# tpfeifle/pointcloud-segmentation-attention

Hardware: AMD Instinct MI355X
Metric: 8192-pt clouds/sec through SA+FP layers, 1/2/4/8 MI355X; HBM GB/s vs peak (higher is better)
Workload: dtype f32

## Files before the change

pointcloud-segmentation-attention_amd/csrc/interp.hip:

```cpp
#include <algorithm>
#include <type_traits>

#include "grid.h"

namespace pn2 {
namespace {

constexpr int kNNBlock = 256;
constexpr int kNNGroup = 4;
constexpr int kNNRows = kNNBlock / kNNGroup;
constexpr int kNNTile = 2048;

struct Best3 {
  float d1, d2, d3;
  int i1, i2, i3;
};

PN2_DEV void best3_init(Best3& b) {
  b.d1 = b.d2 = b.d3 = __builtin_inff();
  b.i1 = b.i2 = b.i3 = 0;
}

PN2_DEV void best3_insert(Best3& b, float d, int k) {
  const bool c1 = d < b.d1, c2 = d < b.d2, c3 = d < b.d3;
  b.d3 = c2 ? b.d2 : (c3 ? d : b.d3);
  b.i3 = c2 ? b.i2 : (c3 ? k : b.i3);
  b.d2 = c1 ? b.d1 : (c2 ? d : b.d2);
  b.i2 = c1 ? b.i1 : (c2 ? k : b.i2);
  b.d1 = c1 ? d : b.d1;
  b.i1 = c1 ? k : b.i1;
}

PN2_DEV bool lex_lt(float d, int k, float bd, int bk) { return d < bd || (d == bd && k < bk); }
PN2_DEV void best3_insert_lex(Best3& b, float d, int k) {
  const bool c1 = lex_lt(d, k, b.d1, b.i1), c2 = lex_lt(d, k, b.d2, b.i2),
             c3 = lex_lt(d, k, b.d3, b.i3);
  b.d3 = c2 ? b.d2 : (c3 ? d : b.d3);
  b.i3 = c2 ? b.i2 : (c3 ? k : b.i3);
  b.d2 = c1 ? b.d1 : (c2 ? d : b.d2);
  b.i2 = c1 ? b.i1 : (c2 ? k : b.i2);
  b.d1 = c1 ? d : b.d1;
  b.i1 = c1 ? k : b.i1;
}

PN2_DEV void best3_merge_xor(Best3& b, int mask) {
  const float d1 = __shfl_xor(b.d1, mask, kWave), d2 = __shfl_xor(b.d2, mask, kWave),
              d3 = __shfl_xor(b.d3, mask, kWave);
  const int i1 = __shfl_xor(b.i1, mask, kWave), i2 = __shfl_xor(b.i2, mask, kWave),
            i3 = __shfl_xor(b.i3, mask, kWave);
  best3_insert_lex(b, d1, i1);
  best3_insert_lex(b, d2, i2);
  best3_insert_lex(b, d3, i3);
}

struct Best3K {
  uint64_t k1, k2, k3;
};
PN2_DEV uint64_t nn_key(float d, int k) {
  return ((uint64_t)__float_as_uint(d) << 32) | (uint32_t)k;
}
PN2_DEV void best3k_init(Best3K& b) { b.k1 = b.k2 = b.k3 = nn_key(__builtin_inff(), 0); }
PN2_DEV void best3k_insert(Best3K& b, uint64_t key) {
  const bool c1 = key < b.k1, c2 = key < b.k2, c3 = key < b.k3;
  b.k3 = c2 ? b.k2 : (c3 ? key : b.k3);
  b.k2 = c1 ? b.k1 : (c2 ? key : b.k2);
  b.k1 = c1 ? key : b.k1;
}
template <int CTRL>
PN2_DEV uint64_t quad_xor_u64(uint64_t v) {
  const uint32_t lo = dpp_u32<CTRL>((uint32_t)v);
  const uint32_t hi = dpp_u32<CTRL>((uint32_t)(v >> 32));
  return ((uint64_t)hi << 32) | lo;
}
template <int CTRL>
PN2_DEV void best3k_merge_quad(Best3K& b) {
  const uint64_t o1 = quad_xor_u64<CTRL>(b.k1), o2 = quad_xor_u64<CTRL>(b.k2),
                 o3 = quad_xor_u64<CTRL>(b.k3);
  best3k_insert(b, o1);
  best3k_insert(b, o2);
  best3k_insert(b, o3);
}
PN2_DEV Best3 best3_of(const Best3K& b) {
  Best3 r;
  r.d1 = __uint_as_float((uint32_t)(b.k1 >> 32));
  r.d2 = __uint_as_float((uint32_t)(b.k2 >> 32));
  r.d3 = __uint_as_float((uint32_t)(b.k3 >> 32));
  r.i1 = (int)(uint32_t)b.k1;
  r.i2 = (int)(uint32_t)b.k2;
  r.i3 = (int)(uint32_t)b.k3;
  return r;
}

PN2_DEV void scan_known(const float* __restrict__ K, int m, float x1, float y1, float z1,
                        float4* sk, Best3& best, int tile = kNNTile) {
  const int q = threadIdx.x & (kNNGroup - 1);
  for (int t0 = 0; t0 < m; t0 += tile) {
    const int cnt = min(tile, m - t0);
    __syncthreads();
    for (int e = threadIdx.x; e < cnt; e += kNNBlock) {
      const float* p = K + 3 * (size_t)(t0 + e);
      sk[e] = make_float4(p[0], p[1], p[2], 0.0f);
    }
    __syncthreads();
#pragma unroll 8
    for (int e = q; e < cnt; e += kNNGroup) {
      const float4 p = sk[e];
      best3_insert(best, sqdist(p.x, p.y, p.z, x1, y1, z1), t0 + e);
    }
  }
  best3_merge_xor(best, 1);
  best3_merge_xor(best, 2);
}

__global__ __launch_bounds__(kNNBlock) void three_nn_kernel(const float* __restrict__ xyz1,
                                                            const float* __restrict__ xyz2, int n,
                                                            int m, float* __restrict__ dist,
                                                            int32_t* __restrict__ idx) {
  __shared__ float4 sk[kNNTile];
  const int b = blockIdx.y;
  const int j = blockIdx.x * kNNRows + threadIdx.x / kNNGroup;
  const bool valid = j < n;
  const float* U = xyz1 + ((size_t)b * n + (valid ? j : 0)) * 3;
  Best3 best;
  best3_init(best);
  scan_known(xyz2 + (size_t)b * m * 3, m, U[0], U[1], U[2], sk, best);
  if (valid && (threadIdx.x & (kNNGroup - 1)) == 0) {
    float* D = dist + ((size_t)b * n + j) * 3;
    int32_t* I = idx + ((size_t)b * n + j) * 3;
    D[0] = best.d1; D[1] = best.d2; D[2] = best.d3;
    I[0] = best.i1; I[1] = best.i2; I[2] = best.i3;
  }
}


PN2_DEV bool box_certifies(const GridHdr& h, float px, float py, float pz, int xl, int xh,
                           int yl, int yh, int zl, int zh, float d3) {
  if (!(d3 < __builtin_inff())) return false;
  const float edge = 1.0f / h.inv;
  float gap = __builtin_inff();
  auto face = [&](float d, float pc, float o, int c) {
    const float fc = o + (float)c * edge;
    gap = fminf(gap, d - 1e-5f * (fabsf(pc) + fabsf(o) + fabsf(fc) + (float)c * edge) - 1e-30f);
  };
  if (xl > 0) face(px - (h.ox + (float)xl * edge), px, h.ox, xl);
  if (xh < h.nx - 1) face((h.ox + (float)(xh + 1) * edge) - px, px, h.ox, xh + 1);
  if (yl > 0) face(py - (h.oy + (float)yl * edge), py, h.oy, yl);
  if (yh < h.ny - 1) face((h.oy + (float)(yh + 1) * edge) - py, py, h.oy, yh + 1);
  if (zl > 0) face(pz - (h.oz + (float)zl * edge), pz, h.oz, zl);
  if (zh < h.nz - 1) face((h.oz + (float)(zh + 1) * edge) - pz, pz, h.oz, zh + 1);
  return gap > 0.0f && d3 < gap * gap * 0.9999f;
}

PN2_DEV float axis_gap(float p, float o, float edge, int c, int cp) {
  if (c == cp) return 0.0f;
  const int f = c > cp ? c : c + 1;
  const float fc = o + (float)f * edge;
  const float d = c > cp ? fc - p : p - fc;
  return fmaxf(d - 1e-5f * (fabsf(p) + fabsf(o) + fabsf(fc) + (float)f * edge) - 1e-30f, 0.0f);
}
PN2_DEV bool gap_excludes(float g2, float d3) { return d3 < g2 * 0.9999f; }

constexpr int kNNFirst = 1;

template <int G, typename Off>
PN2_DEV Best3 grid_nn3(const GridHdr& h, const float4* __restrict__ pts,
                       const Off* __restrict__ off, float px, float py, float pz, int q) {
  Best3K best;
  best3k_init(best);
  auto merged = [&]() {
    Best3K mb = best;
    if constexpr (G == 4) {
      best3k_merge_quad<kDppXor1>(mb);
      best3k_merge_quad<kDppXor2>(mb);
    }
    return best3_of(mb);
  };
  const int cx = cell_coord(px, h.ox, h.inv, h.nx);
  const int cy = cell_coord(py, h.oy, h.inv, h.ny);
  const int cz = cell_coord(pz, h.oz, h.inv, h.nz);
  Best3 res;
  for (int s = kNNFirst;; ++s) {
    const int xl = cx - s, xh = cx + s, yl = cy - s, yh = cy + s, zl = cz - s, zh = cz + s;
    const int x0 = max(xl, 0), x1 = min(xh, h.nx - 1);
    const bool block = s == kNNFirst;
    auto visit = [&](int lo, int hi) {
      for (int e = lo + q; e < hi; e += G) {
        const float4 p = pts[e];
        best3k_insert(best, nn_key(sqdist(p.x, p.y, p.z, px, py, pz), __float_as_int(p.w)));
      }
    };
    if (block) {
      for (int z = max(zl, 0); z <= min(zh, h.nz - 1); ++z)
        for (int y = max(yl, 0); y <= min(yh, h.ny - 1); ++y) {
          const int row = (z * h.ny + y) * h.nx;
          visit(off[row + x0], off[row + x1 + 1]);
        }
    } else {
      const float d3 = res.d3, edge = 1.0f / h.inv;
#pragma nounroll
      for (int z = max(zl, 0); z <= min(zh, h.nz - 1); ++z) {
        const float gz = axis_gap(pz, h.oz, edge, z, cz), gz2 = gz * gz;
        if (gap_excludes(gz2, d3)) continue;
#pragma nounroll
        for (int y = max(yl, 0); y <= min(yh, h.ny - 1); ++y) {
          const float gy = axis_gap(py, h.oy, edge, y, cy), gyz = gz2 + gy * gy;
          if (gap_excludes(gyz, d3)) continue;
          const int row = (z * h.ny + y) * h.nx;
          const bool face = z == zl || z == zh || y == yl || y == yh;
          int xa = face ? x0 : xl, xb = face ? x1 : xh;
#pragma nounroll
          while (xa <= xb) {
            const float g = axis_gap(px, h.ox, edge, xa, cx);
            if (xa >= 0 && xa < h.nx && !gap_excludes(gyz + g * g, d3)) break;
            xa = face || xa != xl ? xa + 1 : xh;
          }
#pragma nounroll
          while (xb > xa) {
            const float g = axis_gap(px, h.ox, edge, xb, cx);
            if (xb >= 0 && xb < h.nx && !gap_excludes(gyz + g * g, d3)) break;
            xb = face || xb != xh ? xb - 1 : xl;
          }
          if (xa > xb) continue;
          if (face || xa == xb) {
            visit(off[row + xa], off[row + xb + 1]);
          } else {
            visit(off[row + xa], off[row + xa + 1]);
            visit(off[row + xb], off[row + xb + 1]);
          }
        }
      }
    }
    res = merged();
    if (xl <= 0 && yl <= 0 && zl <= 0 && xh >= h.nx - 1 && yh >= h.ny - 1 && zh >= h.nz - 1)
      break;
    if (box_certifies(h, px, py, pz, xl, xh, yl, yh, zl, zh, res.d3)) break;
  }
  return res;
}

template <int G, typename Off>
PN2_DEV Best3 grid_nn3_wave(const GridHdr& h, const float4* __restrict__ pts,
                            const Off* __restrict__ off, float px, float py, float pz, int q,
                            bool valid) {
  if (valid) return grid_nn3<G, Off>(h, pts, off, px, py, pz, q);
  Best3 none;
  best3_init(none);
  return none;
}


template <int BLOCK, bool LDS, int G, int K>
__global__ __launch_bounds__(BLOCK) void three_nn_grid_kernel(
    const void* __restrict__ kgrid, int m, const void* __restrict__ ugrid,
    const float* __restrict__ xyz1, int n, int B, float* __restrict__ dist,
    int32_t* __restrict__ idx) {
  static_assert(G == 1 || G == 4, "one lane or a quad per unknown");
  constexpr int QPB = BLOCK / G;
  extern __shared__ float4 s_pts[];
  const int R = (n + QPB * K - 1) / (QPB * K);
  const int Lg = xcd_block(blockIdx.x, R * B);
  if (Lg >= R * B) return;
  const int b = Lg / R;
  const int q = (int)threadIdx.x & (G - 1);
  const GridView g = grid_view(kgrid, b, m);
  const GridHdr& h = g.h;
  const float4* __restrict__ pts = g.pts;
  const int* __restrict__ off = g.off;
  if (LDS && h.ncell <= max(m, kAutoMinCells)) {
    int* s_off = (int*)(s_pts + m);
    for (int e = threadIdx.x; e < m; e += BLOCK) s_pts[e] = g.pts[e];
    for (int e = threadIdx.x; e <= h.ncell; e += BLOCK) s_off[e] = g.off[e];
    __syncthreads();
    pts = s_pts;
    off = s_off;
  }
  const float4* __restrict__ upts = ugrid ? grid_view(ugrid, b, n).pts : nullptr;
  for (int kb = 0; kb < K; ++kb) {
    const int i0 = ((Lg - b * R) * K + kb) * QPB;
    if (i0 >= n) break;
    const int i = i0 + (int)threadIdx.x / G;
    const bool valid = i < n;
    const int ic = valid ? i : n - 1;
    float px, py, pz;
    int u;
    if (upts) {
      const float4 U = upts[ic];
      px = U.x; py = U.y; pz = U.z;
      u = __float_as_int(U.w);
    } else {
      const float* U = xyz1 + ((size_t)b * n + ic) * 3;
      px = U[0]; py = U[1]; pz = U[2];
      u = ic;
    }
    const Best3 res = grid_nn3_wave<G, int>(h, pts, off, px, py, pz, q, valid);
    if (valid && q == 0) {
      float* D = dist + ((size_t)b * n + u) * 3;
      int32_t* I = idx + ((size_t)b * n + u) * 3;
      D[0] = res.d1; D[1] = res.d2; D[2] = res.d3;
      I[0] = res.i1; I[1] = res.i2; I[2] = res.i3;
    }
  }
}

__global__ void idw_kernel(const float* __restrict__ dist, int total, float* __restrict__ weight) {
  const int i = blockIdx.x * blockDim.x + threadIdx.x;
  if (i >= total) return;
  const float* d = dist + 3 * (size_t)i;
  float w1, w2, w3;
  idw(d[0], d[1], d[2], w1, w2, w3);
  weight[3 * (size_t)i + 0] = w1;
  weight[3 * (size_t)i + 1] = w2;
  weight[3 * (size_t)i + 2] = w3;
}

constexpr int kBlock = 256;
constexpr int kTileElems = 2048;

__global__ __launch_bounds__(kBlock) void three_interp_kernel(
    const float* __restrict__ points, const int32_t* __restrict__ idx,
    const float* __restrict__ weight, int m, int C, int n, int rows, FastDiv div_c,
    FastDiv div_n, uint32_t total_rows, float* __restrict__ out) {
  const uint32_t r0 = blockIdx.x * (uint32_t)rows;
  const int nrows = (int)min((uint32_t)rows, total_rows - r0);
  const int elems = nrows * C;
  for (int e = threadIdx.x; e < elems; e += kBlock) {
    const uint32_t rl = fdiv((uint32_t)e, div_c);
    const int c = e - (int)rl * C;
    const uint32_t r = r0 + rl;
    const uint32_t b = fdiv(r, div_n);
    const int32_t* I = idx + 3 * (size_t)r;
    const float* W = weight + 3 * (size_t)r;
    const float* P = points + (size_t)b * m * C + c;
    float v = P[(size_t)I[0] * C] * W[0];
    v = v + P[(size_t)I[1] * C] * W[1];
    v = v + P[(size_t)I[2] * C] * W[2];
    out[(size_t)r * C + c] = v;
  }
}

__global__ __launch_bounds__(kBlock) void three_interp_grad_kernel(
    const float* __restrict__ grad_out, const int32_t* __restrict__ idx,
    const float* __restrict__ weight, int m, int C, int rows, FastDiv div_c, FastDiv div_n,
    uint32_t total_rows, float* __restrict__ grad_points) {
  const uint32_t r0 = blockIdx.x * (uint32_t)rows;
  const int nrows = (int)min((uint32_t)rows, total_rows - r0);
  const int elems = nrows * C;
  for (int e = threadIdx.x; e < elems; e += kBlock) {
    const uint32_t rl = fdiv((uint32_t)e, div_c);
    const int c = e - (int)rl * C;
    const uint32_t r = r0 + rl;
    const uint32_t b = fdiv(r, div_n);
    const int32_t* I = idx + 3 * (size_t)r;
    const float* W = weight + 3 * (size_t)r;
    float* G = grad_points + (size_t)b * m * C + c;
    const float g = grad_out[(size_t)r * C + c];
    atomicAdd(G + (size_t)I[0] * C, g * W[0]);
    atomicAdd(G + (size_t)I[1] * C, g * W[1]);
    atomicAdd(G + (size_t)I[2] * C, g * W[2]);
  }
}

struct FpLayer {
  const float* xyz1;
  const float* xyz2;
  const float* pdist;
  const int32_t* pidx;
  const void* ugrid;
  const float* points1;
  const float* points2;
  float* out;
  int C1, C2, n, m, cw, B, Z;
  FastDiv div_cw;
};

struct FpRow {
  int4 I;
  float4 W;
  int r;
};

template <int V2, int V1, int UN, int FB = kNNBlock, typename RowFn>
PN2_DEV void fp_write_rows(const FpLayer& p, int b, int zb, int j0, RowFn row) {
  const float* __restrict__ points1 = p.points1;
  const float* __restrict__ points2 = p.points2;
  float* __restrict__ out = p.out;
  const int C1 = p.C1, C2 = p.C2, n = p.n, m = p.m, cw = p.cw;
  const FastDiv div_cw = p.div_cw;
  const int Cout = C2 + C1;
  const int c2v = C2 / V2, coutv = c2v + C1 / V1;
  const int cb = zb * cw;
  const int ce = min(coutv, cb + cw);
  if (ce <= cb) return;
  const int nrows = min(FB / kNNGroup, n - j0);
  const int elems = nrows * cw;
  using V2T = typename std::conditional<V2 == 4, float4, float>::type;
  using V1T = typename std::conditional<
      V1 == 4, float4, typename std::conditional<V1 == 2, float2, float>::type>::type;
  const V2T* P2 = reinterpret_cast<const V2T*>(points2 + (size_t)b * m * C2);
  const float* P1 = points1 + (size_t)b * n * C1;
  float* O = out + (size_t)b * n * Cout;
  constexpr int U = UN;
  for (int e0 = threadIdx.x; e0 < elems; e0 += FB * U) {
    V2T a[U], bb[U], cc[U];
    V1T q[U];
    float4 W[U];
    bool cat[U], ok[U];
    size_t o[U];
#pragma unroll
    for (int u = 0; u < U; ++u) {
      const int e = e0 + u * FB;
      const int rl = (int)fdiv((uint32_t)(e < elems ? e : e0), div_cw);
      int c = cb + ((e < elems ? e : e0) - rl * cw);
      ok[u] = e < elems && c < ce;
      c = min(c, ce - 1);
      const FpRow rw = row(rl);
      const int r = rw.r;
      cat[u] = c >= c2v;
      W[u] = rw.W;
      if constexpr (V1 == V2) {
        const int4 I = rw.I;
        const V2T* P1v = reinterpret_cast<const V2T*>(P1);
        const V2T* pa = cat[u] ? P1v + (size_t)r * (C1 / V1) + (c - c2v) : P2 + (size_t)I.x * c2v + c;
        const V2T* pb = cat[u] ? pa : P2 + (size_t)I.y * c2v + c;
        const V2T* pc = cat[u] ? pa : P2 + (size_t)I.z * c2v + c;
        a[u] = *pa;
        bb[u] = *pb;
        cc[u] = *pc;
        q[u] = V1T{};
        o[u] = (size_t)r * Cout + (size_t)c * V2;
      } else if (!cat[u]) {
        q[u] = V1T{};
        const int4 I = rw.I;
        a[u] = P2[(size_t)I.x * c2v + c];
        bb[u] = P2[(size_t)I.y * c2v + c];
        cc[u] = P2[(size_t)I.z * c2v + c];
        o[u] = (size_t)r * Cout + (size_t)c * V2;
      } else {
        q[u] = *reinterpret_cast<const V1T*>(P1 + (size_t)r * C1 + (size_t)(c - c2v) * V1);
        a[u] = bb[u] = cc[u] = V2T{};
        o[u] = (size_t)r * Cout + C2 + (size_t)(c - c2v) * V1;
      }
    }
#pragma unroll
    for (int u = 0; u < U; ++u) {
      if (!ok[u]) continue;
      if constexpr (V1 == V2) {
        const bool k = cat[u];
        if constexpr (V2 == 4) {
          float4 v;
          v.x = k ? a[u].x : (a[u].x * W[u].x + bb[u].x * W[u].y) + cc[u].x * W[u].z;
          v.y = k ? a[u].y : (a[u].y * W[u].x + bb[u].y * W[u].y) + cc[u].y * W[u].z;
          v.z = k ? a[u].z : (a[u].z * W[u].x + bb[u].z * W[u].y) + cc[u].z * W[u].z;
          v.w = k ? a[u].w : (a[u].w * W[u].x + bb[u].w * W[u].y) + cc[u].w * W[u].z;
          *reinterpret_cast<float4*>(O + o[u]) = v;
        } else {
          O[o[u]] = k ? a[u] : (a[u] * W[u].x + bb[u] * W[u].y) + cc[u] * W[u].z;
        }
        continue;
      }
      if (cat[u]) {
        *reinterpret_cast<V1T*>(O + o[u]) = q[u];
        continue;
      }
      if constexpr (V2 == 4) {
        float4 v;
        v.x = (a[u].x * W[u].x + bb[u].x * W[u].y) + cc[u].x * W[u].z;
        v.y = (a[u].y * W[u].x + bb[u].y * W[u].y) + cc[u].y * W[u].z;
        v.z = (a[u].z * W[u].x + bb[u].z * W[u].y) + cc[u].z * W[u].z;
        v.w = (a[u].w * W[u].x + bb[u].w * W[u].y) + cc[u].w * W[u].z;
        if (V1 == 4 || (o[u] & 3) == 0) {
          *reinterpret_cast<float4*>(O + o[u]) = v;
        } else if (V1 == 2) {
          *reinterpret_cast<float2*>(O + o[u]) = make_float2(v.x, v.y);
          *reinterpret_cast<float2*>(O + o[u] + 2) = make_float2(v.z, v.w);
        } else {
          O[o[u]] = v.x;
          O[o[u] + 1] = v.y;
          O[o[u] + 2] = v.z;
          O[o[u] + 3] = v.w;
        }
      } else {
        O[o[u]] = (a[u] * W[u].x + bb[u] * W[u].y) + cc[u] * W[u].z;
      }
    }
  }
}

template <int V2, int V1, bool PRE, int UN>
PN2_DEV void fp_fused_body(const FpLayer& p, int Lg, float4* sk, int tile) {
  __shared__ int4 s_idx[kNNRows];
  __shared__ float4 s_w[kNNRows];
  __shared__ int s_row[PRE ? kNNRows : 1];
  const float* __restrict__ xyz1 = p.xyz1;
  const float* __restrict__ xyz2 = p.xyz2;
  const float* __restrict__ pdist = p.pdist;
  const int32_t* __restrict__ pidx = p.pidx;
  const void* __restrict__ ugrid = p.ugrid;
  const int n = p.n, m = p.m, Z = p.Z;
  const int R = (n + kNNRows - 1) / kNNRows;
  const int b = Lg / (R * Z);
  const int zb = (Lg - b * R * Z) / R;
  const int j0 = (Lg - b * R * Z - zb * R) * kNNRows;
  if constexpr (PRE) {
    int jj = j0 + (int)threadIdx.x;
    if (threadIdx.x < kNNRows && jj < n) {
      if (ugrid) jj = __float_as_int(grid_view(ugrid, b, n).pts[jj].w);
      s_row[threadIdx.x] = jj;
      const float* D = pdist + ((size_t)b * n + jj) * 3;
      const int32_t* I = pidx + ((size_t)b * n + jj) * 3;
      float w1, w2, w3;
      idw(D[0], D[1], D[2], w1, w2, w3);
      s_idx[threadIdx.x] = make_int4(I[0], I[1], I[2], 0);
      s_w[threadIdx.x] = make_float4(w1, w2, w3, 0.0f);
    }
  } else {
    const int jl = threadIdx.x / kNNGroup;
    const int j = j0 + jl;
    const bool valid = j < n;
    const float* U = xyz1 + ((size_t)b * n + (valid ? j : 0)) * 3;
    Best3 best;
    best3_init(best);
    scan_known(xyz2 + (size_t)b * m * 3, m, U[0], U[1], U[2], sk, best, tile);
    if ((threadIdx.x & (kNNGroup - 1)) == 0) {
      float w1, w2, w3;
      idw(best.d1, best.d2, best.d3, w1, w2, w3);
      s_idx[jl] = make_int4(best.i1, best.i2, best.i3, 0);
      s_w[jl] = make_float4(w1, w2, w3, 0.0f);
    }
  }
  __syncthreads();
  fp_write_rows<V2, V1, UN>(p, b, zb, j0, [&](int rl) {
    if constexpr (PRE) return FpRow{s_idx[rl], s_w[rl], s_row[rl]};
    else return FpRow{s_idx[rl], s_w[rl], j0 + rl};
  });
}

template <int V2, int V1, bool PRE, int UN>
__global__ __launch_bounds__(kNNBlock) void fp_fused_kernel(FpLayer p, int tile) {
  extern __shared__ float4 sk[];
  const int total = (p.n + kNNRows - 1) / kNNRows * p.B * p.Z;
  const int Lg = xcd_block(blockIdx.x, total);
  if (Lg >= total) return;
  fp_fused_body<V2, V1, PRE, UN>(p, Lg, sk, tile);
}

constexpr int kFpGridMaxKnown = PN2_FP_GRID_MAX_KNOWN;
constexpr float kFpgPointsPerCell = 2.0f;
constexpr int kFpgBlock = 256;
#ifndef PN2_FPG_STAMP
#define PN2_FPG_STAMP 0
#endif
#if PN2_FPG_STAMP
__device__ unsigned long long g_fpg_stamp[4096 * 8];
#define PN2_FPG_T(K) if (t == 0 && Lg < 4096) g_fpg_stamp[Lg * 8 + (K)] = __builtin_amdgcn_s_memtime();
#else
#define PN2_FPG_T(K)
#endif

size_t device_lds_per_block() {
  static size_t cache[64] = {0};
  int dev = 0;
  if (hipGetDevice(&dev) != hipSuccess || dev < 0 || dev >= 64) return 64 * 1024;
  if (!cache[dev]) {
    int v = 0, o = 0;
    if (hipDeviceGetAttribute(&v, hipDeviceAttributeMaxSharedMemoryPerBlock, dev) != hipSuccess)
      v = 0;
    if (hipDeviceGetAttribute(&o, hipDeviceAttributeSharedMemPerBlockOptin, dev) != hipSuccess)
      o = 0;
    v = std::max(v, o);
    if (v <= 0) return 64 * 1024;
    cache[dev] = (size_t)v;
  }
  return cache[dev];
}

inline size_t fp_grid_lds(int m) {
  const size_t cells = (size_t)ceil((double)m * kAutoPointsPerCell / kFpgPointsPerCell);
  return (size_t)m * 16 + ((std::max(cells, (size_t)kAutoMinCells) + 1) * 2 + 3) / 4 * 4;
}

template <int V2, int V1, int UN, int KPT, int FB>
__global__ __launch_bounds__(FB) void fp_grid_fused_kernel(FpLayer p, float* __restrict__ dist,
                                                        int32_t* __restrict__ idx,
                                                        const char* __restrict__ kgrid) {
  constexpr int NW = FB / kWave;
  constexpr int FR = FB / kNNGroup;
  extern __shared__ float4 s_pts[];
  __shared__ int4 s_idx[FR];
  __shared__ float s_wv[3][FR];
  float(*red)[NW] = reinterpret_cast<float(*)[NW]>(&s_wv[0][0]);
  int* wsum = reinterpret_cast<int*>(&s_wv[1][0]);
  GridHdr* shp = reinterpret_cast<GridHdr*>(&s_wv[2][0]);
  static_assert(6 * NW <= FR && sizeof(GridHdr) <= FR * 4, "build scratch fits");
  const int n = p.n, m = p.m;
  const int R = (n + FR - 1) / FR;
  const int total = R * p.B;
  const int Lg = xcd_block(blockIdx.x, total);
  if (Lg >= total) return;
  const int b = Lg / R;
  const int j0 = (Lg - b * R) * FR;
  const int t = threadIdx.x, lane = t & (kWave - 1), w = t / kWave;
  uint16_t* s_off = reinterpret_cast<uint16_t*>(s_pts + m);
  uint32_t* s_cnt = reinterpret_cast<uint32_t*>(s_pts + m);
  PN2_FPG_T(0)
  GridHdr h;
  bool built = false;
  if (kgrid) {
    const char* G = kgrid + (size_t)b * grid_stride(m);
    h = *reinterpret_cast<const GridHdr*>(G);
    if (h.ncell >= 1 && h.ncell <= max(m, kAutoMinCells)) {
      const int* goff = reinterpret_cast<const int*>(G + sizeof(GridHdr));
      const float4* gpts = reinterpret_cast<const float4*>(G + kGridOffBytes);
      for (int i = t; i < m; i += FB) s_pts[i] = gpts[i];
      for (int i = t; i <= h.ncell; i += FB) s_off[i] = (uint16_t)goff[i];
      __syncthreads();
      built = true;
    }
  }
  if (!built) {
    const float* __restrict__ K = p.xyz2 + (size_t)b * m * 3;
    float mn[3] = {INFINITY, INFINITY, INFINITY}, mx[3] = {-INFINITY, -INFINITY, -INFINITY};
#pragma unroll
    for (int i = 0; i < KPT; ++i) {
      const int k = t + i * FB;
      if (k < m) {
#pragma unroll
        for (int a = 0; a < 3; ++a) {
          const float v = K[3 * k + a];
          mn[a] = fminf(mn[a], v);
          mx[a] = fmaxf(mx[a], v);
        }
      }
    }
#pragma unroll
    for (int a = 0; a < 3; ++a) {
      mn[a] = wave_min_f(mn[a]);
      mx[a] = wave_max_f(mx[a]);
    }
    if (lane == 0) {
#pragma unroll
      for (int a = 0; a < 3; ++a) { red[a][w] = mn[a]; red[3 + a][w] = mx[a]; }
    }
    __syncthreads();
    if (t == 0) {
      float lo[3], hi[3];
      for (int a = 0; a < 3; ++a) {
        lo[a] = red[a][0];
        hi[a] = red[3 + a][0];
        for (int i = 1; i < NW; ++i) { lo[a] = fminf(lo[a], red[a][i]); hi[a] = fmaxf(hi[a], red[3 + a][i]); }
        if (!(hi[a] >= lo[a])) { lo[a] = 0.0f; hi[a] = 0.0f; }
      }
      *shp = grid_dims(lo, hi, m, 0.0f, kFpgPointsPerCell);
    }
    __syncthreads();
    h = *shp;
    PN2_FPG_T(1)
    auto cell_at = [&](float x, float y, float z) {
      const int ix = cell_coord(x, h.ox, h.inv, h.nx);
      const int iy = cell_coord(y, h.oy, h.inv, h.ny);
      const int iz = cell_coord(z, h.oz, h.inv, h.nz);
      return (iz * h.ny + iy) * h.nx + ix;
    };

    for (int i = t; i < (h.ncell + 2) / 2; i += FB) s_cnt[i] = 0u;
    __syncthreads();
    int kc[KPT], kr[KPT];
#pragma unroll
    for (int i = 0; i < KPT; ++i) {
      const int k = t + i * FB;
      kc[i] = 0;
      kr[i] = 0;
      if (k < m) {
        const int c = cell_at(K[3 * k + 0], K[3 * k + 1], K[3 * k + 2]);
        const int sh = 16 * (c & 1);
        const uint32_t old = atomicAdd(&s_cnt[c >> 1], 1u << sh);
        kc[i] = c;
        kr[i] = (int)((old >> sh) & 0xFFFFu);
      }
    }
    __syncthreads();
    {
      const int per = (h.ncell + FB - 1) / FB;
      const int s0 = t * per, s1 = min(s0 + per, h.ncell);
      int sum = 0;
      for (int i = s0; i < s1; ++i) sum += s_off[i];
      const int incl = wave_incl_scan(sum, lane);
      if (lane == kWave - 1) wsum[w] = incl;
      __syncthreads();
      int base = incl - sum;
      for (int i = 0; i < w; ++i) base += wsum[i];
      for (int i = s0; i < s1; ++i) {
        const int c = s_off[i];
        s_off[i] = (uint16_t)base;
        base += c;
      }
      if (t == 0) s_off[h.ncell] = (uint16_t)m;
    }
    __syncthreads();
#pragma unroll
    for (int i = 0; i < KPT; ++i) {
      const int k = t + i * FB;
      if (k < m)
        s_pts[s_off[kc[i]] + kr[i]] = make_float4(K[3 * k + 0], K[3 * k + 1], K[3 * k + 2],
                                                  __int_as_float(k));
    }
    __syncthreads();
  }

  PN2_FPG_T(2)
  const int jl = t / kNNGroup, q = t & (kNNGroup - 1);
  const int j = j0 + jl;
  {
    const bool valid = j < n;
    const int jc = valid ? j : n - 1;
    float px, py, pz;
    int u;
    if (p.ugrid) {
      const float4 U = grid_view(p.ugrid, b, n).pts[jc];
      px = U.x; py = U.y; pz = U.z;
      u = __float_as_int(U.w);
    } else {
      const float* U = p.xyz1 + ((size_t)b * n + jc) * 3;
      px = U[0]; py = U[1]; pz = U[2];
      u = jc;
    }
    const Best3 res = grid_nn3_wave<kNNGroup, uint16_t>(h, s_pts, s_off, px, py, pz, q, valid);
    if (valid && q == 0) {
      float w1, w2, w3;
      idw(res.d1, res.d2, res.d3, w1, w2, w3);
      s_idx[jl] = make_int4(res.i1, res.i2, res.i3, u);
      s_wv[0][jl] = w1;
      s_wv[1][jl] = w2;
      s_wv[2][jl] = w3;
      if (dist) {
        float* D = dist + ((size_t)b * n + u) * 3;
        int32_t* I = idx + ((size_t)b * n + u) * 3;
        D[0] = res.d1; D[1] = res.d2; D[2] = res.d3;
        I[0] = res.i1; I[1] = res.i2; I[2] = res.i3;
      }
    }
  }
  __syncthreads();
  PN2_FPG_T(3)
  fp_write_rows<V2, V1, UN, FB>(p, b, 0, j0, [&](int rl) {
    const int4 I = s_idx[rl];
    return FpRow{I, make_float4(s_wv[0][rl], s_wv[1][rl], s_wv[2][rl], 0.0f), I.w};
  });
  PN2_FPG_T(4)
}

constexpr int kFpMaxLayers = PN2_FP_MAX_LAYERS;
struct FpLayers {
  FpLayer l[kFpMaxLayers];
  int first[kFpMaxLayers + 1];
  int nlayers, B;
};
template <int V2, int V1, bool PRE, int UN>
__global__ __launch_bounds__(kNNBlock) void fp_fused_layers_kernel(FpLayers a, int tile) {
  extern __shared__ float4 sk[];
  const int per_cloud_all = a.first[a.nlayers];
  const int total = per_cloud_all * a.B;
  const int L = xcd_block(blockIdx.x, total);
  if (L >= total) return;
  const int b = L / per_cloud_all;
  const int lc = L - b * per_cloud_all;
  int li = 0;
  while (li + 1 < a.nlayers && lc >= a.first[li + 1]) ++li;
  const int per_cloud = a.first[li + 1] - a.first[li];
  fp_fused_body<V2, V1, PRE, UN>(a.l[li], b * per_cloud + (lc - a.first[li]), sk, tile);
}

int batch_chunk(int B, int n, int C, int rows) {
  if ((long long)rows * C * C >= (1LL << 32)) return 0;
  long long per_b = (long long)n * n;
  if (per_b >= (1LL << 32)) return 0;
  long long ch = ((1LL << 32) - 1) / (per_b > 0 ? per_b : 1);
  if ((long long)n * ch >= (1LL << 31)) ch = ((1LL << 31) - 1) / (n > 0 ? n : 1);
  return (int)(ch < B ? ch : B);
}

constexpr int kFpMinBlocks = 512;
constexpr int kFpMinCols = 16;
constexpr int kFpScanBudget = 4096;

struct FpPlan {
  FpLayer p;
  int v2, v1, pre, blocks;
};

int fp_plan(const float* xyz1, const float* xyz2, const float* pdist, const int32_t* pidx,
            const void* ugrid, const float* points1, int C1, const float* points2, int C2,
            int B, int n, int m, float* out, FpPlan& f, bool split = true) {
  const bool pre = pdist != nullptr;
  const bool v2 = C2 % 4 == 0 && aligned16(points2, out);
  const int v1 = !v2 ? 1
                 : C1 % 4 == 0 && aligned16(points1) ? 4
                 : C1 % 2 == 0 && (((uintptr_t)points1 & 7) == 0) ? 2 : 1;
  const int coutv = C2 / (v2 ? 4 : 1) + C1 / v1;
  const int row_blocks = (n + kNNRows - 1) / kNNRows;
  int zsplit = 1;
  while (split && (long long)row_blocks * B * zsplit < kFpMinBlocks &&
         coutv / (zsplit * 2) >= kFpMinCols &&
         (pre || (long long)m * zsplit * 2 <= kFpScanBudget))
    zsplit *= 2;
  const int cw = (coutv + zsplit - 1) / zsplit;
  if ((long long)kNNRows * cw * cw >= (1LL << 32)) return PN2_EINVAL;
  if ((long long)row_blocks * B * zsplit >= (1LL << 31) - 8) return PN2_EINVAL;
  f.p = FpLayer{xyz1, xyz2, pdist, pidx, ugrid, points1, points2, out,
                C1, C2, n, m, cw, B, zsplit, make_fastdiv((uint32_t)cw)};
  f.v2 = v2;
  f.v1 = v1;
  f.pre = pre;
  f.blocks = row_blocks * B * zsplit;
  return PN2_OK;
}

constexpr int kFpUnroll = 2;
#define PN2_FP_DISPATCH(KERNEL, f, arg, blocks, MAXM, stream)                                  \
  do {                                                                                         \
    const dim3 grid__(xcd_grid(blocks));                                                       \
    const int tile__ = std::max(1, std::min((int)(MAXM), kNNTile));                            \
    if ((f).v1 == 4) { PN2_FP_PRE(KERNEL, 4, 4, f, arg, grid__, tile__, stream); }             \
    else if ((f).v1 == 2) { PN2_FP_PRE(KERNEL, 4, 2, f, arg, grid__, tile__, stream); }        \
    else if ((f).v2) { PN2_FP_PRE(KERNEL, 4, 1, f, arg, grid__, tile__, stream); }             \
    else { PN2_FP_PRE(KERNEL, 1, 1, f, arg, grid__, tile__, stream); }                         \
  } while (0)
#define PN2_FP_PRE(KERNEL, V2, V1, f, arg, grid, tile, stream)                                 \
  if ((f).pre) hipLaunchKernelGGL((KERNEL<V2, V1, true, kFpUnroll>), grid, dim3(kNNBlock), 0, stream, arg, tile); \
  else hipLaunchKernelGGL((KERNEL<V2, V1, false, kFpUnroll>), grid, dim3(kNNBlock), (size_t)(tile) * sizeof(float4), stream, arg, tile)

int fp_launch(const float* xyz1, const float* xyz2, const float* pdist, const int32_t* pidx,
              const void* ugrid, const float* points1, int C1, const float* points2, int C2,
              int B, int n, int m, float* out, hipStream_t stream) {
  FpPlan f;
  const int rc = fp_plan(xyz1, xyz2, pdist, pidx, ugrid, points1, C1, points2, C2, B, n, m, out, f);
  if (rc != PN2_OK) return rc;
  PN2_FP_DISPATCH(fp_fused_kernel, f, f.p, f.blocks, m, stream);
  PN2_RETURN_LAUNCH();
}

int fp_grid_launch(const float* xyz1, const float* xyz2, const void* ugrid, const float* points1,
                   int C1, const float* points2, int C2, int B, int n, int m, float* out,
                   float* dist, int32_t* idx, const void* kgrid, hipStream_t stream) {
  FpPlan f;
  const int rc = fp_plan(xyz1, xyz2, nullptr, nullptr, ugrid, points1, C1, points2, C2, B, n, m,
                         out, f, false);
  if (rc != PN2_OK) return rc;
  const dim3 grid(xcd_grid((long long)((n + kFpgBlock / kNNGroup - 1) / (kFpgBlock / kNNGroup)) *
                           B)),
      blk(kFpgBlock);
  const size_t lds = fp_grid_lds(m);
  constexpr int FR = kFpgBlock / kNNGroup;
  if (lds + 28 * FR + 64 > device_lds_per_block()) return PN2_ENOTSUP;
  if ((long long)FR * f.p.cw * f.p.cw >= (1LL << 32)) return PN2_EINVAL;
  const char* kg = (const char*)kgrid;
#define PN2_FPG_K(V2, V1, U)                                                                   \
  if (m <= 4 * kFpgBlock) hipLaunchKernelGGL((fp_grid_fused_kernel<V2, V1, U, 4, kFpgBlock>), grid, blk, lds, stream, f.p, dist, idx, kg); \
  else hipLaunchKernelGGL((fp_grid_fused_kernel<V2, V1, U, (kFpGridMaxKnown + kFpgBlock - 1) / kFpgBlock, kFpgBlock>), grid, blk, lds, stream, f.p, dist, idx, kg)
#define PN2_FPG(V2, V1) PN2_FPG_K(V2, V1, kFpUnroll);
  if (f.v1 == 4) { PN2_FPG(4, 4) }
  else if (f.v1 == 2) { PN2_FPG(4, 2) }
  else if (f.v2) { PN2_FPG(4, 1) }
  else { PN2_FPG(1, 1) }
#undef PN2_FPG
#undef PN2_FPG_K
  PN2_RETURN_LAUNCH();
}

int fp_layers_launch(const pn2_fp_layer* layers, int nlayers, int B, hipStream_t stream) {
  if (!layers || nlayers < 1 || nlayers > PN2_FP_MAX_LAYERS || B < 0 || B > 65535)
    return PN2_EINVAL;
  FpLayers a{};
  FpPlan f0{};
  long long blocks = 0;
  int nl = 0, maxm = 0;
  for (int i = 0; i < nlayers; ++i) {
    const pn2_fp_layer& s = layers[i];
    if (s.n < 0 || s.m < 0 || s.C1 < 0 || s.C2 < 0) return PN2_EINVAL;
    if (!s.points1 && s.C1 != 0) return PN2_EINVAL;
    if ((long long)B * s.n == 0 || s.C1 + s.C2 == 0) continue;
    if (!s.xyz1 || !s.out || (s.m > 0 && !s.xyz2) || (s.C2 > 0 && !s.points2)) return PN2_EINVAL;
    if (s.m == 0 && s.C2 > 0) return PN2_EINVAL;
    FpPlan f;
    const int rc = fp_plan(s.xyz1, s.xyz2, nullptr, nullptr, nullptr, s.points1, s.C1,
                                s.points2, s.C2, B, s.n, s.m, s.out, f);
    if (rc != PN2_OK) return rc;
    if (nl == 0) f0 = f;
    if (f.v2 != f0.v2 || f.v1 != f0.v1) {
      PN2_FP_DISPATCH(fp_fused_kernel, f, f.p, f.blocks, s.m, stream);
      const hipError_t e = hipGetLastError();
      if (e != hipSuccess) return (int)e;
      continue;
    }
    a.l[nl] = f.p;
    maxm = std::max(maxm, s.m);
    a.first[nl] = (int)blocks;
    blocks += f.blocks / B;
    ++nl;
  }
  if (nl == 0) return PN2_OK;
  a.first[nl] = (int)blocks;
  a.nlayers = nl;
  a.B = B;
  PN2_FP_DISPATCH(fp_fused_layers_kernel, f0, a, blocks * B, maxm, stream);
  PN2_RETURN_LAUNCH();
}

}
}

extern "C" {

int pn2_three_nn(const float* xyz1, const float* xyz2, int B, int n, int m, float* dist,
                 int32_t* idx, pn2_stream_t stream) {
  if (B < 0 || n < 0 || m < 0 || B > 65535) return PN2_EINVAL;
  if ((long long)B * n == 0) return PN2_OK;
  if (!xyz1 || !dist || !idx || (m > 0 && !xyz2)) return PN2_EINVAL;
  hipLaunchKernelGGL(pn2::three_nn_kernel, dim3((n + pn2::kNNRows - 1) / pn2::kNNRows, B),
                     dim3(pn2::kNNBlock), 0, (hipStream_t)stream, xyz1, xyz2, n, m, dist, idx);
  PN2_RETURN_LAUNCH();
}

int pn2_idw_weights(const float* dist, int B, int n, float* weight, pn2_stream_t stream) {
  if (B < 0 || n < 0) return PN2_EINVAL;
  const long long total = (long long)B * n;
  if (total == 0) return PN2_OK;
  if (total > INT32_MAX || !dist || !weight) return PN2_EINVAL;
  hipLaunchKernelGGL(pn2::idw_kernel, dim3((unsigned)((total + 255) / 256)), dim3(256), 0,
                     (hipStream_t)stream, dist, (int)total, weight);
  PN2_RETURN_LAUNCH();
}

int pn2_three_interpolate(const float* points, const int32_t* idx, const float* weight, int B,
                          int m, int C, int n, float* out, pn2_stream_t stream) {
  if (B < 0 || m < 0 || C < 0 || n < 0) return PN2_EINVAL;
  if ((long long)B * n == 0 || C == 0) return PN2_OK;
  if (!points || !idx || !weight || !out) return PN2_EINVAL;
  const int rows = C >= pn2::kTileElems ? 1 : pn2::kTileElems / C;
  const int chunk = pn2::batch_chunk(B, n, C, rows);
  if (chunk <= 0) return PN2_EINVAL;
  for (int b0 = 0; b0 < B; b0 += chunk) {
    const int nb = B - b0 < chunk ? B - b0 : chunk;
    const long long total_rows = (long long)nb * n;
    const long long tiles = (total_rows + rows - 1) / rows;
    hipLaunchKernelGGL(pn2::three_interp_kernel, dim3((unsigned)tiles), dim3(pn2::kBlock), 0,
                       (hipStream_t)stream, points + (size_t)b0 * m * C, idx + (size_t)b0 * n * 3,
                       weight + (size_t)b0 * n * 3, m, C, n, rows, pn2::make_fastdiv((uint32_t)C),
                       pn2::make_fastdiv((uint32_t)n), (uint32_t)total_rows,
                       out + (size_t)b0 * n * C);
    hipError_t e = hipGetLastError();
    if (e != hipSuccess) return (int)e;
  }
  return PN2_OK;
}

int pn2_three_interpolate_grad(const float* grad_out, const int32_t* idx, const float* weight,
                               int B, int n, int C, int m, float* grad_points,
                               pn2_stream_t stream) {
  if (B < 0 || m < 0 || C < 0 || n < 0) return PN2_EINVAL;
  const size_t bytes = (size_t)B * m * C * sizeof(float);
  if (bytes) {
    if (!grad_points) return PN2_EINVAL;
    hipError_t e = hipMemsetAsync(grad_points, 0, bytes, (hipStream_t)stream);
    if (e != hipSuccess) return (int)e;
  }
  if ((long long)B * n == 0 || C == 0) return PN2_OK;
  if (!grad_out || !idx || !weight) return PN2_EINVAL;
  const int rows = C >= pn2::kTileElems ? 1 : pn2::kTileElems / C;
  const int chunk = pn2::batch_chunk(B, n, C, rows);
  if (chunk <= 0) return PN2_EINVAL;
  for (int b0 = 0; b0 < B; b0 += chunk) {
    const int nb = B - b0 < chunk ? B - b0 : chunk;
    const long long total_rows = (long long)nb * n;
    const long long tiles = (total_rows + rows - 1) / rows;
    hipLaunchKernelGGL(pn2::three_interp_grad_kernel, dim3((unsigned)tiles), dim3(pn2::kBlock), 0,
                       (hipStream_t)stream, grad_out + (size_t)b0 * n * C,
                       idx + (size_t)b0 * n * 3, weight + (size_t)b0 * n * 3, m, C, rows,
                       pn2::make_fastdiv((uint32_t)C), pn2::make_fastdiv((uint32_t)n),
                       (uint32_t)total_rows, grad_points + (size_t)b0 * m * C);
    hipError_t e = hipGetLastError();
    if (e != hipSuccess) return (int)e;
  }
  return PN2_OK;
}

int pn2_fp_fused(const float* xyz1, const float* xyz2, const float* points1, int C1,
                 const float* points2, int C2, int B, int n, int m, float* out,
                 pn2_stream_t stream) {
  if (B < 0 || n < 0 || m < 0 || C1 < 0 || C2 < 0 || B > 65535) return PN2_EINVAL;
  if (!points1 && C1 != 0) return PN2_EINVAL;
  if ((long long)B * n == 0 || C1 + C2 == 0) return PN2_OK;
  if (!xyz1 || !out || (m > 0 && !xyz2) || (C2 > 0 && !points2)) return PN2_EINVAL;
  if (m == 0 && C2 > 0) return PN2_EINVAL;
  return pn2::fp_launch(xyz1, xyz2, nullptr, nullptr, nullptr, points1, C1, points2, C2, B, n,
                        m, out, (hipStream_t)stream);
}

int pn2_fp_fused_layers(const pn2_fp_layer* layers, int nlayers, int B, pn2_stream_t stream) {
  return pn2::fp_layers_launch(layers, nlayers, B, (hipStream_t)stream);
}

int pn2_fp_apply(const float* dist, const int32_t* idx, const void* unknown_grid,
                 const float* points1, int C1, const float* points2, int C2, int B, int n, int m,
                 float* out, pn2_stream_t stream) {
  if (B < 0 || n < 0 || m < 0 || C1 < 0 || C2 < 0 || B > 65535) return PN2_EINVAL;
  if (!points1 && C1 != 0) return PN2_EINVAL;
  if ((long long)B * n == 0 || C1 + C2 == 0) return PN2_OK;
  if (!dist || !idx || !out || (C2 > 0 && !points2)) return PN2_EINVAL;
  if (m == 0 && C2 > 0) return PN2_EINVAL;
  return pn2::fp_launch(nullptr, nullptr, dist, idx, unknown_grid, points1, C1, points2, C2, B,
                        n, m, out, (hipStream_t)stream);
}

int pn2_fp_grid_fused(const float* xyz1, const float* xyz2, const void* unknown_grid,
                      const float* points1, int C1, const float* points2, int C2, int B, int n,
                      int m, float* out, float* dist, int32_t* idx, pn2_stream_t stream) {
  if (B < 0 || n < 0 || m < 1 || m > pn2::kFpGridMaxKnown || C1 < 0 || C2 < 0 || B > 65535)
    return PN2_EINVAL;
  if (!points1 && C1 != 0) return PN2_EINVAL;
  if ((dist == nullptr) != (idx == nullptr)) return PN2_EINVAL;
  if ((long long)B * n == 0) return PN2_OK;
  if (C1 + C2 == 0) return dist ? PN2_EINVAL : PN2_OK;
  if (!xyz2 || (!xyz1 && !unknown_grid) || !out || (C2 > 0 && !points2))
    return PN2_EINVAL;
  return pn2::fp_grid_launch(xyz1, xyz2, unknown_grid, points1, C1, points2, C2, B, n, m, out,
                             dist, idx, nullptr, (hipStream_t)stream);
}

#if PN2_FPG_STAMP
int pn2_fpg_stamps(unsigned long long* host_out) {
  return (int)hipMemcpyFromSymbol(host_out, HIP_SYMBOL(pn2::g_fpg_stamp),
                                  sizeof(unsigned long long) * 4096 * 8, 0,
                                  hipMemcpyDeviceToHost);
}
#endif

int pn2_fp_grid_fused_known(const void* known_grid, const float* xyz1, const float* xyz2,
                            const void* unknown_grid, const float* points1, int C1,
                            const float* points2, int C2, int B, int n, int m, float* out,
                            float* dist, int32_t* idx, pn2_stream_t stream) {
  if (!known_grid || !pn2::aligned16(known_grid)) return PN2_EINVAL;
  if (B < 0 || n < 0 || m < 1 || m > pn2::kFpGridMaxKnown || C1 < 0 || C2 < 0 || B > 65535)
    return PN2_EINVAL;
  if (!points1 && C1 != 0) return PN2_EINVAL;
  if ((dist == nullptr) != (idx == nullptr)) return PN2_EINVAL;
  if ((long long)B * n == 0) return PN2_OK;
  if (C1 + C2 == 0) return dist ? PN2_EINVAL : PN2_OK;
  if (!xyz2 || (!xyz1 && !unknown_grid) || !out || (C2 > 0 && !points2))
    return PN2_EINVAL;
  return pn2::fp_grid_launch(xyz1, xyz2, unknown_grid, points1, C1, points2, C2, B, n, m, out,
                             dist, idx, known_grid, (hipStream_t)stream);
}

int pn2_three_nn_grid(const void* known_grid, const void* unknown_grid, const float* xyz1,
                      int B, int n, int m, float* dist, int32_t* idx, pn2_stream_t stream) {
  if (B < 0 || n < 0 || m < 0 || B > 65535) return PN2_EINVAL;
  if ((long long)B * n == 0) return PN2_OK;
  if (!known_grid || !dist || !idx || (!unknown_grid && !xyz1)) return PN2_EINVAL;
  constexpr int BLOCK = 256;
  if ((long long)((n + BLOCK / 4 - 1) / (BLOCK / 4)) * B >= (1LL << 31) - 8) return PN2_EINVAL;
  const size_t lds = (size_t)m * 16 + (size_t)(std::max(m, pn2::kAutoMinCells) + 1) * 4;
  constexpr int G = 4, K = 1;
  const dim3 grid(pn2::xcd_grid((long long)((n + BLOCK / G * K - 1) / (BLOCK / G * K)) * B));
  if (lds <= 64 * 1024)
    hipLaunchKernelGGL((pn2::three_nn_grid_kernel<BLOCK, true, G, K>), grid, dim3(BLOCK), lds,
                       (hipStream_t)stream, known_grid, m, unknown_grid, xyz1, n, B, dist, idx);
  else
    hipLaunchKernelGGL((pn2::three_nn_grid_kernel<BLOCK, false, G, K>), grid, dim3(BLOCK), 0,
                       (hipStream_t)stream, known_grid, m, unknown_grid, xyz1, n, B, dist, idx);
  PN2_RETURN_LAUNCH();
}

}
```

Baseline: 103,800.

## Start 3-NN grid search with the nearest 2x2x2 octant before the full block

The grid 3-NN search now first scans only the 2x2x2 octant of cells nearest to the query point and returns early if the box certificate proves the three nearest are found. Otherwise it scans the remaining cells of the 3x3x3 block with per-row gap pruning, skipping the already visited octant, and then falls back to the expanding shell loop. This aims to cut candidate point visits in dense grids, at the cost of an extra merge/certify step and more branching per query. Optional counting instrumentation and a points-per-cell macro are also added, both inactive by default.

```diff
diff --git a/pointcloud-segmentation-attention_amd/csrc/interp.hip b/pointcloud-segmentation-attention_amd/csrc/interp.hip
--- a/pointcloud-segmentation-attention_amd/csrc/interp.hip
+++ b/pointcloud-segmentation-attention_amd/csrc/interp.hip
@@ -162,9 +162,33 @@
 
 constexpr int kNNFirst = 1;
 
+#ifndef PN2_NN_OCTANT
+#define PN2_NN_OCTANT 1
+#endif
+constexpr bool kNNOctant = PN2_NN_OCTANT != 0;
+static_assert(!kNNOctant || kNNFirst == 1, "the octant is a corner of the 3x3x3 block");
+
+#ifndef PN2_FPG_STAMP
+#define PN2_FPG_STAMP 0
+#endif
+#if PN2_FPG_STAMP >= 2
+struct NnCount {
+  uint32_t cand, octant, block, later;
+};
+#define PN2_NN_CNT(X) do { if (cnt) { X; } } while (0)
+#else
+struct NnCount;
+#define PN2_NN_CNT(X)
+#endif
+
+[[maybe_unused]] PN2_DEV int near_side(float p, float o, float inv, int c) {
+  return (p - o) * inv - (float)c >= 0.5f ? 1 : -1;
+}
+
 template <int G, typename Off>
 PN2_DEV Best3 grid_nn3(const GridHdr& h, const float4* __restrict__ pts,
-                       const Off* __restrict__ off, float px, float py, float pz, int q) {
+                       const Off* __restrict__ off, float px, float py, float pz, int q,
+                       NnCount* cnt = nullptr) {
   Best3K best;
   best3k_init(best);
   auto merged = [&]() {
@@ -175,20 +199,76 @@
     }
     return best3_of(mb);
   };
+  auto visit = [&](int lo, int hi) {
+    for (int e = lo + q; e < hi; e += G) {
+      const float4 p = pts[e];
+      best3k_insert(best, nn_key(sqdist(p.x, p.y, p.z, px, py, pz), __float_as_int(p.w)));
+      PN2_NN_CNT(++cnt->cand);
+    }
+  };
+  auto covers = [&](int xl, int xh, int yl, int yh, int zl, int zh) {
+    return xl <= 0 && yl <= 0 && zl <= 0 && xh >= h.nx - 1 && yh >= h.ny - 1 && zh >= h.nz - 1;
+  };
   const int cx = cell_coord(px, h.ox, h.inv, h.nx);
   const int cy = cell_coord(py, h.oy, h.inv, h.ny);
   const int cz = cell_coord(pz, h.oz, h.inv, h.nz);
   Best3 res;
-  for (int s = kNNFirst;; ++s) {
+  int s = kNNFirst;
+  if constexpr (kNNOctant) {
+    const int sx = near_side(px, h.ox, h.inv, cx), sy = near_side(py, h.oy, h.inv, cy),
+              sz = near_side(pz, h.oz, h.inv, cz);
+    const int xl = min(cx, cx + sx), xh = max(cx, cx + sx), yl = min(cy, cy + sy),
+              yh = max(cy, cy + sy), zl = min(cz, cz + sz), zh = max(cz, cz + sz);
+    {
+      const int x0 = max(xl, 0), x1 = min(xh, h.nx - 1);
+      for (int z = max(zl, 0); z <= min(zh, h.nz - 1); ++z)
+        for (int y = max(yl, 0); y <= min(yh, h.ny - 1); ++y) {
+          const int row = (z * h.ny + y) * h.nx;
+          visit(off[row + x0], off[row + x1 + 1]);
+        }
+    }
+    res = merged();
+    if (covers(xl, xh, yl, yh, zl, zh) ||
+        box_certifies(h, px, py, pz, xl, xh, yl, yh, zl, zh, res.d3)) {
+      PN2_NN_CNT(cnt->octant = 1);
+      return res;
+    }
+    const float d3 = res.d3, edge = 1.0f / h.inv;
+#pragma nounroll
+    for (int z = max(cz - 1, 0); z <= min(cz + 1, h.nz - 1); ++z) {
+      const float gz = axis_gap(pz, h.oz, edge, z, cz), gz2 = gz * gz;
+      if (gap_excludes(gz2, d3)) continue;
+#pragma nounroll
+      for (int y = max(cy - 1, 0); y <= min(cy + 1, h.ny - 1); ++y) {
+        const float gy = axis_gap(py, h.oy, edge, y, cy), gyz = gz2 + gy * gy;
+        if (gap_excludes(gyz, d3)) continue;
+        const bool inner = z >= zl && z <= zh && y >= yl && y <= yh;
+        int xa = inner ? cx - sx : cx - 1, xb = inner ? cx - sx : cx + 1;
+        if (xa < cx) {
+          const float g = axis_gap(px, h.ox, edge, cx - 1, cx);
+          if (xa < 0 || gap_excludes(gyz + g * g, d3)) xa = cx;
+        }
+        if (xb > cx) {
+          const float g = axis_gap(px, h.ox, edge, cx + 1, cx);
+          if (xb > h.nx - 1 || gap_excludes(gyz + g * g, d3)) xb = cx;
+        }
+        if (xa > xb) continue;
+        const int row = (z * h.ny + y) * h.nx;
+        visit(off[row + xa], off[row + xb + 1]);
+      }
+    }
+    res = merged();
+    if (covers(cx - 1, cx + 1, cy - 1, cy + 1, cz - 1, cz + 1) ||
+        box_certifies(h, px, py, pz, cx - 1, cx + 1, cy - 1, cy + 1, cz - 1, cz + 1, res.d3)) {
+      PN2_NN_CNT(cnt->block = 1);
+      return res;
+    }
+    s = kNNFirst + 1;
+  }
+  for (;; ++s) {
     const int xl = cx - s, xh = cx + s, yl = cy - s, yh = cy + s, zl = cz - s, zh = cz + s;
     const int x0 = max(xl, 0), x1 = min(xh, h.nx - 1);
-    const bool block = s == kNNFirst;
-    auto visit = [&](int lo, int hi) {
-      for (int e = lo + q; e < hi; e += G) {
-        const float4 p = pts[e];
-        best3k_insert(best, nn_key(sqdist(p.x, p.y, p.z, px, py, pz), __float_as_int(p.w)));
-      }
-    };
+    const bool block = !kNNOctant && s == kNNFirst;
     if (block) {
       for (int z = max(zl, 0); z <= min(zh, h.nz - 1); ++z)
         for (int y = max(yl, 0); y <= min(yh, h.ny - 1); ++y) {
@@ -231,18 +311,19 @@
       }
     }
     res = merged();
-    if (xl <= 0 && yl <= 0 && zl <= 0 && xh >= h.nx - 1 && yh >= h.ny - 1 && zh >= h.nz - 1)
+    if (covers(xl, xh, yl, yh, zl, zh) ||
+        box_certifies(h, px, py, pz, xl, xh, yl, yh, zl, zh, res.d3))
       break;
-    if (box_certifies(h, px, py, pz, xl, xh, yl, yh, zl, zh, res.d3)) break;
-  }
+  }
+  PN2_NN_CNT(if (!kNNOctant && s == kNNFirst) cnt->block = 1; else cnt->later = 1);
   return res;
 }
 
 template <int G, typename Off>
 PN2_DEV Best3 grid_nn3_wave(const GridHdr& h, const float4* __restrict__ pts,
                             const Off* __restrict__ off, float px, float py, float pz, int q,
-                            bool valid) {
-  if (valid) return grid_nn3<G, Off>(h, pts, off, px, py, pz, q);
+                            bool valid, NnCount* cnt = nullptr) {
+  if (valid) return grid_nn3<G, Off>(h, pts, off, px, py, pz, q, cnt);
   Best3 none;
   best3_init(none);
   return none;
@@ -545,11 +626,11 @@
 }
 
 constexpr int kFpGridMaxKnown = PN2_FP_GRID_MAX_KNOWN;
-constexpr float kFpgPointsPerCell = 2.0f;
+#ifndef PN2_FPG_PPC
+#define PN2_FPG_PPC 2.0f
+#endif
+constexpr float kFpgPointsPerCell = PN2_FPG_PPC;
 constexpr int kFpgBlock = 256;
-#ifndef PN2_FPG_STAMP
-#define PN2_FPG_STAMP 0
-#endif
 #if PN2_FPG_STAMP
 __device__ unsigned long long g_fpg_stamp[4096 * 8];
 #define PN2_FPG_T(K) if (t == 0 && Lg < 4096) g_fpg_stamp[Lg * 8 + (K)] = __builtin_amdgcn_s_memtime();
@@ -724,7 +805,28 @@
       px = U[0]; py = U[1]; pz = U[2];
       u = jc;
     }
+#if PN2_FPG_STAMP >= 2
+    __shared__ unsigned int s_nnc[4];
+    if (t < 4) s_nnc[t] = 0u;
+    __syncthreads();
+    NnCount nc = {0u, 0u, 0u, 0u};
+    const Best3 res =
+        grid_nn3_wave<kNNGroup, uint16_t>(h, s_pts, s_off, px, py, pz, q, valid, &nc);
+    atomicAdd(&s_nnc[0], nc.cand);
+    if (q == 0) {
+      atomicAdd(&s_nnc[1], nc.octant);
+      atomicAdd(&s_nnc[2], nc.block);
+      atomicAdd(&s_nnc[3], nc.later);
+    }
+    __syncthreads();
+    if (t == 0 && Lg < 4096) {
+      g_fpg_stamp[Lg * 8 + 5] = s_nnc[0];
+      g_fpg_stamp[Lg * 8 + 6] = s_nnc[1];
+      g_fpg_stamp[Lg * 8 + 7] = (unsigned long long)s_nnc[2] | ((unsigned long long)s_nnc[3] << 32);
+    }
+#else
     const Best3 res = grid_nn3_wave<kNNGroup, uint16_t>(h, s_pts, s_off, px, py, pz, q, valid);
+#endif
     if (valid && q == 0) {
       float w1, w2, w3;
       idw(res.d1, res.d2, res.d3, w1, w2, w3);
```

New measurement: 104,700 (median of 6 runs). No clear change (+0.8%).
